# MP-ReID/mp-reid

Hardware: AMD Instinct MI355X
Metric: gallery images/s encode + distmat+rerank ms, 20k×20k; mAP/Rank-1 parity (higher is better)
Workload: dtype f16 pairs hi+lo (3 MFMA products per multiply-add, f32-grade), f32 acc; distmat f32 exact; 1 GPU; Market-1501 configs[1]: do_inference ViT-B/16 3368q+15913g/GPU, no rerank; HBM-resident loader; encoder_batch=508, encoder_precision=split, encoder_streams=2, rerank=False, distance_mode=exact

## Files before the change

mp-reid_amd/csrc/api.cpp:

```cpp
#include "common.h"

#include <cstring>
#include <string>
#include <utility>
#include <vector>

static thread_local char g_err[512] = "";

void mpreid_set_error(const char *fmt, ...) {
    va_list ap;
    va_start(ap, fmt);
    vsnprintf(g_err, sizeof(g_err), fmt, ap);
    va_end(ap);
}

namespace {
struct TuneTable {
    std::vector<std::pair<std::string, int>> kv;
    TuneTable() {
        static const char *known[] = {"gemm_big", "gemm_stagger", "gemm_stagger_all", "jaccard_wave", "jaccard_wave_rows",
                                      "jaccard_table", "csc_atomic", "rerank_overlap", "dist_sym_p2", "dist_sym_p2_naps", "dist_sym_p2_abl", "dist_sym_p2_grid", "dist_sym_p2_strip", "dist_p2_full", "gemm_walk", "gemm_grid", "gemm_ragged", "wide_sort_lds", "wide_jaccard_rows", "verbose"};
        const char *e = getenv("MPREID_TUNE");
        if (!e) return;
        std::string s(e);
        size_t pos = 0;
        while (pos <= s.size()) {
            size_t end = s.find(',', pos);
            if (end == std::string::npos) end = s.size();
            std::string item = s.substr(pos, end - pos);
            pos = end + 1;
            if (item.empty()) continue;
            const size_t eq = item.find('=');
            const std::string key = item.substr(0, eq);
            const int val = eq == std::string::npos ? 1 : atoi(item.c_str() + eq + 1);
            bool ok = false;
            for (const char *k : known) ok = ok || key == k;
            if (!ok) fprintf(stderr, "[mpreid] MPREID_TUNE: unknown key '%s' ignored\n", key.c_str());
            else kv.emplace_back(key, val);
        }
    }
};
}

int mpreid_tune(const char *key, int dflt) {
// ... 41 lines not shown
```

mp-reid_amd/csrc/gemm_f16.hip:

```cpp
#include <algorithm>
#include <cstdlib>
#include <type_traits>

#include "gemm_f16.h"

typedef __attribute__((address_space(3))) void lds_ptr_t;
typedef const __attribute__((address_space(1))) void glb_ptr_t;

__device__ __forceinline__ void dma16(const void *gsrc, unsigned char *lds_dst_wave_base) {
    __builtin_amdgcn_global_load_lds((glb_ptr_t *)gsrc, (lds_ptr_t *)lds_dst_wave_base, 16, 0, 0);
}

__device__ __forceinline__ unsigned lds_addr(const void *p) {
    return (unsigned)(uintptr_t)(const __attribute__((address_space(3))) void *)p;
}
__device__ __forceinline__ void dma16_sv(uint64_t sbase, unsigned voff, unsigned lds_dst) {
    unsigned keep;
    asm volatile("s_mov_b32 %0, m0\n\t"
                 "s_mov_b32 m0, %3\n\t"
                 "s_nop 0\n\t"
                 "global_load_lds_dwordx4 %2, %1 nt\n\t"
                 "s_mov_b32 m0, %0"
                 : "=&s"(keep)
                 : "s"(sbase), "v"(voff), "s"(lds_dst)
// ... 427 lines not shown
                            reinterpret_cast<float *>(g.out)[((int64_t)b * g.L + 1 + p) * g.ldo + n] =
                                a + g.aux[(int64_t)(1 + p) * g.N + n];
                        }
                    } else if (EPI == GE_COSINE) {
                        if (m < g.m_valid && n < g.n_valid) {
                            const float sc = g.rscale ? g.rscale[m] * g.cscale[n] : 1.0f;
                            float c = (a * sc) * __fdiv_rn(1.0f, g.aux[m] * bnv);
                            const float lo = (float)(-1.0 + 0.00001), hi = (float)(1.0 - 0.00001);
                            c = c < lo ? lo : (c > hi ? hi : c);
                            reinterpret_cast<float *>(g.out)[(int64_t)m * g.ldo + n] = acosf(c);
                        }
                    }
                }
        }
    }
}

constexpr int BBM = 256, BBN = 256, BBK = 32, B_NSTAGE = 4;
constexpr int B_PART_BYTES = BBM * BBK * 2;
constexpr int B_STAGE_BYTES = 2 * B_PART_BYTES;
constexpr int B_LDS_BYTES = B_NSTAGE * B_STAGE_BYTES;
constexpr int B_LDS_TOTAL = B_LDS_BYTES + 8 * 4096;

template <int EPI, int DBG = 0, bool SYM = false>
__global__ __launch_bounds__(512) void gemm_f16_big_kernel(GemmArgs g, int tiles_m, int tiles_n) {
    extern __shared__ __attribute__((aligned(16))) unsigned char smem[];
    const int tid = threadIdx.x, lane = tid & 63;
    const int wave = __builtin_amdgcn_readfirstlane(tid >> 6);
    const int wr = wave >> 2, wc = wave & 3;
    const int K = g.K;
    constexpr bool SPLIT = gemm_epi_is_split(EPI);
    constexpr bool SYM_STORE = (EPI == GE_EUCLID) && SYM;
    constexpr bool SYM_EPI = (EPI == GE_CAND) || SYM_STORE;
    const int nseg = SPLIT ? g.kseg / BBK : 0;
    const int nst = SPLIT ? 3 * nseg : K / BBK;
    auto koff_a = [&](int st) -> int {
        if constexpr (!SPLIT) return st * BBK;
        const int r = st / 3, sidx = st - 3 * r;
        return sidx == 0 ? r * BBK : (sidx == 1 ? g.kseg + r * BBK : -1);
    };
    auto koff_b = [&](int st) -> int {
        if constexpr (!SPLIT) return st * BBK;
        const int r = st / 3, sidx = st - 3 * r;
        return sidx == 0 ? r * BBK : (sidx == 2 ? g.kseg + r * BBK : -1);
    };

    const int ntiles = tiles_m * tiles_n;
// ... 179 lines not shown
                const unsigned fl = rw >> 28, row = rw & 0x0fffffffu;
                if (fl & 1u) {
                    const unsigned p = atomicAdd(&g.cnt_lo[row], 1u);
                    if (p < (unsigned)g.cap_lo) g.list_lo[(size_t)row * g.cap_lo + p] = make_uint2(cw, dv);
                }
                if (fl & 2u) {
                    const unsigned p = atomicAdd(&g.cnt_hi[row], 1u);
                    if (p < (unsigned)g.cap_hi) g.list_hi[(size_t)row * g.cap_hi + p] = make_uint2(cw, dv);
                }
                if (fl & 4u) {
                    const unsigned p = atomicAdd(&g.cnt_lo[cw], 1u);
                    if (p < (unsigned)g.cap_lo) g.list_lo[(size_t)cw * g.cap_lo + p] = make_uint2(row, dv);
                }
                if (fl & 8u) {
                    const unsigned p = atomicAdd(&g.cnt_hi[cw], 1u);
                    if (p < (unsigned)g.cap_hi) g.list_hi[(size_t)cw * g.cap_hi + p] = make_uint2(row, dv);
                }
            }
            __builtin_amdgcn_wave_barrier();
            cl_n = 0;
        }
    };

    int tile = tile_at(pos);
    if (tile < 0) return;
    if (g.stagger > 0) {
        const unsigned long long t0 = __builtin_amdgcn_s_memrealtime();
        const unsigned long long wait = g.stagger_mode ? (unsigned long long)g.stagger * ((blockIdx.x >> 3) & 7u) / 8u
                                                       : (unsigned long long)g.stagger * (blockIdx.x & 255u) / 256u;
        while (__builtin_amdgcn_s_memrealtime() - t0 < wait) __builtin_amdgcn_s_sleep(32);
    }
    set_tile(tile);
    dma_prologue();
    [[maybe_unused]] int stamp_tile = 0;
    for (;;) {
    f32x4 acc[8][4];
#pragma unroll
    for (int i = 0; i < 8; ++i)
#pragma unroll
        for (int j = 0; j < 4; ++j) acc[i][j] = f32x4{0.f, 0.f, 0.f, 0.f};

    if constexpr (SPLIT) asm volatile("s_waitcnt vmcnt(4)\n\ts_barrier" ::: "memory");
    else if constexpr (PAIR) {
        if (nst > 2) asm volatile("s_waitcnt vmcnt(8)\n\ts_barrier" ::: "memory");
        else asm volatile("s_waitcnt vmcnt(0)\n\ts_barrier" ::: "memory");
    } else if (nst > 2) asm volatile("s_waitcnt vmcnt(8)\n\ts_barrier" ::: "memory");
    else asm volatile("s_waitcnt vmcnt(4)\n\ts_barrier" ::: "memory");

    auto stamp = [&](int which) {
        if constexpr ((DBG & 32) != 0) {
            if (g.stamps && tid == 0 && stamp_tile < 32)
                g.stamps[((size_t)blockIdx.x * 32 + stamp_tile) * 8 + which] = __builtin_amdgcn_s_memrealtime();
        }
    };
    stamp(0);
    f16x8 fa0[8], fb0[4], fa1[8], fb1[4];
    load_frags(0, fa0, fb0);

    auto mfma32 = [&](f16x8 (&fa)[8], f16x8 (&fb)[4]) {
#pragma unroll
        for (int i = 0; i < 8; ++i)
#pragma unroll
            for (int j = 0; j < 4; ++j)
                acc[i][j] = __builtin_amdgcn_mfma_f32_16x16x32_f16(fa[i], fb[j], acc[i][j], 0, 0, 0);
    };
// ... 55 lines not shown
                else asm volatile("s_waitcnt vmcnt(0)\n\ts_barrier" ::: "memory");
            } else {
                if (t + 2 < nst) asm volatile("s_waitcnt vmcnt(4)\n\ts_barrier" ::: "memory");
                else asm volatile("s_waitcnt vmcnt(0)\n\ts_barrier" ::: "memory");
                if (t + 3 < nst) dma_stage(t + 3);
            }
            load_frags(t + 1, na, nb);
        }
        mfma32(fa, fb);
    };
    if constexpr (SPLIT) {
        auto sstep = [&](auto S_, auto TAIL_, int t) {
            constexpr int S = decltype(S_)::value;
            constexpr bool TAIL = decltype(TAIL_)::value;
            constexpr int s0 = S % 3;
            constexpr bool ldA = s0 != 1, ldB = s0 != 0;
            constexpr bool dmA = s0 != 2, dmB = s0 != 1;
            f16x8 (&fa)[8] = (S & 1) ? fa1 : fa0;
            f16x8 (&fb)[4] = (s0 == 2) ? fb1 : fb0;
            f16x8 (&na)[8] = (S < 3) ? fa1 : fa0;
            f16x8 (&nb)[4] = (s0 == 1) ? fb1 : fb0;
            constexpr bool more1 = !TAIL || S < 5, more3 = !TAIL || S < 3;
            if constexpr (more1) {
                if constexpr (TAIL && S >= 4) asm volatile("s_waitcnt vmcnt(0)\n\ts_barrier" ::: "memory");
                else if constexpr (s0 == 1) asm volatile("s_waitcnt vmcnt(4)\n\ts_barrier" ::: "memory");
                else asm volatile("s_waitcnt vmcnt(2)\n\ts_barrier" ::: "memory");
            }
            unsigned char *dbase = smem + ((t + 3) & (B_NSTAGE - 1)) * B_STAGE_BYTES + wave * 2048;
            const unsigned char *sb = smem + ((t + 1) & (B_NSTAGE - 1)) * B_STAGE_BYTES;
            const int r3 = (t + 3) / 3;
            const int koff = (s0 == 1 ? g.kseg : 0) + r3 * BBK, koffb = (s0 == 2 ? g.kseg : 0) + r3 * BBK;
            auto piece = [&](int q) {
                if (!more3) return;
                if (dmA && q < 2) dma16(a_src + (int64_t)(q * 16) * K + koff, dbase + q * 1024);
                else if (dmB && q - (dmA ? 2 : 0) >= 0 && q - (dmA ? 2 : 0) < 2)
                    dma16(b_src + (int64_t)((q - (dmA ? 2 : 0)) * 16) * K + koffb, dbase + B_PART_BYTES + (q - (dmA ? 2 : 0)) * 1024);
            };
            auto rd_a = [&](int i) { if (more1) na[i] = *reinterpret_cast<const f16x8 *>(sb + a_off + i * 1024); };
            auto rd_b = [&](int j) { if (more1) nb[j] = *reinterpret_cast<const f16x8 *>(sb + b_off + j * 1024); };
#pragma unroll
            for (int gq = 0; gq < 4; ++gq) {
                piece(gq);
                if constexpr (ldA && ldB) {
                    if (gq == 0) { rd_b(0); rd_b(1); rd_b(2); }
                    if (gq == 1) { rd_b(3); rd_a(0); rd_a(1); }
                    if (gq == 2) { rd_a(2); rd_a(3); rd_a(4); }
                    if (gq == 3) { rd_a(5); rd_a(6); rd_a(7); }
// ... 24 lines not shown
        sstep(integral_constant<int, 0>{}, integral_constant<bool, true>{}, t);
        sstep(integral_constant<int, 1>{}, integral_constant<bool, true>{}, t + 1);
        sstep(integral_constant<int, 2>{}, integral_constant<bool, true>{}, t + 2);
        sstep(integral_constant<int, 3>{}, integral_constant<bool, true>{}, t + 3);
        sstep(integral_constant<int, 4>{}, integral_constant<bool, true>{}, t + 4);
        sstep(integral_constant<int, 5>{}, integral_constant<bool, true>{}, t + 5);
    } else {
    int t = 0;
    for (; t + 4 < nst; t += 2) {
        step_steady(std::integral_constant<int, 0>{}, t, fa0, fb0, fa1, fb1);
        step_steady(std::integral_constant<int, 1>{}, t + 1, fa1, fb1, fa0, fb0);
    }
    for (; t < nst; t += 2) {
        step_tail(t, fa0, fb0, fa1, fb1);
        step_tail(t + 1, fa1, fb1, fa0, fb0);
    }
    }

    __syncthreads();
    stamp(1);
    const int cur_m0 = m0, cur_n0 = n0;
    pos += pos_step;
    const int next_tile = tile_at(pos);
    unsigned char *patch = smem + B_LDS_BYTES;
    if constexpr (DBG & 8) {
#pragma unroll
        for (int i = 0; i < 8; ++i)
#pragma unroll
            for (int j = 0; j < 4; ++j) asm volatile("" ::"v"(acc[i][j]));
    } else if constexpr (EPI == GE_CAND) {
        const bool mirror = g.sym != 0 && cur_m0 != cur_n0;
        float *tp = reinterpret_cast<float *>(smem + wave * 16384);
        const int rb = cur_m0 + wr * 128, cb = cur_n0 + wc * 64;
        const float NEG = -__builtin_huge_valf(), POS = __builtin_huge_valf();
        float *rt = tp + 1024;
        float *ct = rt + 384;
        {
            const float a0 = g.aux[rb + lane], a1 = g.aux[rb + 64 + lane];
            const float l0 = g.tlo[rb + lane], l1 = g.tlo[rb + 64 + lane];
            const float h0 = g.thi[rb + lane], h1 = g.thi[rb + 64 + lane];
            const int c = cb + lane;
            const bool cv = c < g.n_valid;
            const float cn = cv ? g.aux2[c] : 0.f;
            const float cl = (mirror && cv) ? g.tlo[c] : NEG, chh = (mirror && cv) ? g.thi[c] : POS;
            rt[lane] = a0; rt[64 + lane] = a1;
            rt[128 + lane] = l0; rt[192 + lane] = l1;
// ... 82 lines not shown
            for (int j = 0; j < 4; ++j)
#pragma unroll
                for (int r = 0; r < 4; ++r) {
                    float v = acc[i][j][r] + bias[j];
                    if (EPI == GE_BIAS_GELU) v = quick_gelu(v);
                    if (EPI == GE_BIAS_RELU) v = v < 0.f ? 0.f : v;
                    wreg[(fq * 4 + r) * 72 + j * 16 + frow] = (_Float16)v;
                }
            __builtin_amdgcn_fence(__ATOMIC_RELEASE, "wavefront");
            __builtin_amdgcn_wave_barrier();
            __builtin_amdgcn_fence(__ATOMIC_ACQUIRE, "wavefront");
#pragma unroll
            for (int it = 0; it < 2; ++it) {
                const int lr = it * 8 + (lane >> 3), ch = lane & 7;
                const uint4 v = *reinterpret_cast<const uint4 *>(wreg + lr * 72 + ch * 8);
                _Float16 *dsth = out + (int64_t)(cur_m0 + wr * 128 + i * 16 + lr) * g.ldo + cur_n0 + wc * 64 + ch * 8;
                if (EPI == GE_BIAS_RELU) *reinterpret_cast<uint4 *>(dsth) = v;
                else store_nt(dsth, v);
            }
            __builtin_amdgcn_wave_barrier();
        }
    } else if constexpr (EPI == GE_S_BIAS_GELU || EPI == GE_S_BIAS_RELU_PAIR) {
        _Float16 *whi = reinterpret_cast<_Float16 *>(patch + wave * 4096);
        _Float16 *wlo = reinterpret_cast<_Float16 *>(smem + wave * 4096);
        _Float16 *out = reinterpret_cast<_Float16 *>(g.out);
        float bias[4];
#pragma unroll
        for (int j = 0; j < 4; ++j) bias[j] = g.bias[cur_n0 + wc * 64 + j * 16 + frow];
#pragma unroll
        for (int i = 0; i < 8; ++i) {
#pragma unroll
            for (int j = 0; j < 4; ++j)
#pragma unroll
                for (int rp = 0; rp < 4; rp += 2) {
                    typedef float f32x2 __attribute__((ext_vector_type(2)));
                    typedef _Float16 f16x2 __attribute__((ext_vector_type(2)));
                    const f32x2 a = {acc[i][j][rp], acc[i][j][rp + 1]};
                    const f32x2 h = __builtin_elementwise_fma(a, f32x2{g.oscale, g.oscale}, f32x2{bias[j], bias[j]});
                    f32x2 v;
                    if constexpr (EPI == GE_S_BIAS_GELU) {
                        const f32x2 t = h * (-1.702f * 1.44269504088896340736f);
                        const f32x2 d = f32x2{__builtin_amdgcn_exp2f(t[0]), __builtin_amdgcn_exp2f(t[1])} + 1.0f;
                        v = h * f32x2{__builtin_amdgcn_rcpf(d[0]), __builtin_amdgcn_rcpf(d[1])};
                    } else {
                        v = f32x2{h[0] < 0.f ? 0.f : h[0], h[1] < 0.f ? 0.f : h[1]};
                    }
                    f16x2 hi, lo;
                    split_pair2(v[0], v[1], hi, lo);
                    whi[(fq * 4 + rp) * 72 + j * 16 + frow] = hi[0];
                    whi[(fq * 4 + rp + 1) * 72 + j * 16 + frow] = hi[1];
                    wlo[(fq * 4 + rp) * 72 + j * 16 + frow] = lo[0];
                    wlo[(fq * 4 + rp + 1) * 72 + j * 16 + frow] = lo[1];
                }
            __builtin_amdgcn_fence(__ATOMIC_RELEASE, "wavefront");
            __builtin_amdgcn_wave_barrier();
            __builtin_amdgcn_fence(__ATOMIC_ACQUIRE, "wavefront");
#pragma unroll
            for (int it = 0; it < 2; ++it) {
                const int lr = it * 8 + (lane >> 3), ch = lane & 7;
                const uint4 vh = *reinterpret_cast<const uint4 *>(whi + lr * 72 + ch * 8);
                const uint4 vl = *reinterpret_cast<const uint4 *>(wlo + lr * 72 + ch * 8);
                _Float16 *dsth = out + (int64_t)(cur_m0 + wr * 128 + i * 16 + lr) * g.ldo + cur_n0 + wc * 64 + ch * 8;
                if constexpr (EPI == GE_S_BIAS_RELU_PAIR) {
                    if (cur_n0 + wc * 64 + ch * 8 < g.pair_c) {
                        *reinterpret_cast<uint4 *>(dsth) = vh;
                        *reinterpret_cast<uint4 *>(dsth + g.pair_c) = vl;
                    }
                } else {
                    store_nt(dsth, vh);
                    store_nt(dsth + g.N, vl);
                }
            }
            __builtin_amdgcn_wave_barrier();
        }
        asm volatile("s_barrier" ::: "memory");
    } else if constexpr (EPI == GE_BIAS_ADD_RELU) {
        _Float16 *wreg = reinterpret_cast<_Float16 *>(patch + wave * 4096);
        _Float16 *pid = reinterpret_cast<_Float16 *>(smem + wave * 4096);
        _Float16 *outh = reinterpret_cast<_Float16 *>(g.out);
        const int nb0 = cur_n0 + wc * 64;
        float bias[4];
#pragma unroll
        for (int j = 0; j < 4; ++j) bias[j] = g.bias[nb0 + j * 16 + frow];
        const int lr0 = lane >> 3, ch = lane & 7;
        auto id_load = [&](int i, int it) -> uint4 {
            return *reinterpret_cast<const uint4 *>(g.identity + (int64_t)(cur_m0 + wr * 128 + i * 16 + it * 8 + lr0) * g.ldo +
                                                    nb0 + ch * 8);
        };
        uint4 idn0 = id_load(0, 0), idn1 = id_load(0, 1);
#pragma unroll
        for (int i = 0; i < 8; ++i) {
            *reinterpret_cast<uint4 *>(pid + lr0 * 72 + ch * 8) = idn0;
            *reinterpret_cast<uint4 *>(pid + (8 + lr0) * 72 + ch * 8) = idn1;
            if (i + 1 < 8) {
                idn0 = id_load(i + 1, 0);
                idn1 = id_load(i + 1, 1);
            }
            __builtin_amdgcn_fence(__ATOMIC_RELEASE, "wavefront");
// ... 91 lines not shown
                store16_sv(x_base(i * 16 + it * 4), x_loff, o);
                if constexpr (EPI == GE_S_BIAS_RES_PAIR) {
                    typedef _Float16 h4p __attribute__((ext_vector_type(4)));
                    h4p hi, lo;
                    {
                        const float y[4] = {o[0] < 0.f ? 0.f : o[0], o[1] < 0.f ? 0.f : o[1], o[2] < 0.f ? 0.f : o[2],
                                            o[3] < 0.f ? 0.f : o[3]};
                        split_pairs<4>(y, hi, lo);
                    }
                    const uint64_t pb = reinterpret_cast<uint64_t>(g.pair_out) +
                                        (uint64_t)(((int64_t)(cur_m0 + wr * 128 + i * 16 + it * 4) * 2 * g.pair_c + nbase) * 2);
                    store8_sv(pb, p_loff, __builtin_bit_cast(u32x2, hi));
                    store8_sv(pb + (uint64_t)g.pair_c * 2u, p_loff, __builtin_bit_cast(u32x2, lo));
                }
            }
            if (i + 4 < 8) x_dma(i + 4);
            __builtin_amdgcn_wave_barrier();
            asm volatile("" ::: "memory");
        }
        asm volatile("s_barrier" ::: "memory");
    } else {
        float *wreg = reinterpret_cast<float *>(patch + wave * 4096);
        float *outp = reinterpret_cast<float *>(g.out);
        const bool vec_ok = (g.ldo % 4 == 0) && ((reinterpret_cast<uintptr_t>(outp) & 15) == 0);
        const int nbase = cur_n0 + wc * 64;
        const int c4 = (lane & 15) * 4;
        float4 bias4 = make_float4(0.f, 0.f, 0.f, 0.f), bn4 = bias4, cs4 = make_float4(1.f, 1.f, 1.f, 1.f);
        float bias1 = 0.f, bnv1 = 0.f, cs1 = 1.f;
        if (EPI == GE_EUCLID && g.rscale) {
            cs4 = *reinterpret_cast<const float4 *>(g.cscale + nbase + c4);
            cs1 = g.cscale[nbase + lane];
        }
        if (vec_ok) {
            if (EPI == GE_BIAS_RES || EPI == GE_S_BIAS_RES || EPI == GE_S_BIAS_RES_PAIR || EPI == GE_S_BIAS_F32)
                bias4 = *reinterpret_cast<const float4 *>(g.bias + nbase + c4);
            if (EPI == GE_EUCLID) {
                bn4.x = (nbase + c4 + 0 < g.n_valid) ? g.aux2[nbase + c4 + 0] : 0.f;
                bn4.y = (nbase + c4 + 1 < g.n_valid) ? g.aux2[nbase + c4 + 1] : 0.f;
                bn4.z = (nbase + c4 + 2 < g.n_valid) ? g.aux2[nbase + c4 + 2] : 0.f;
                bn4.w = (nbase + c4 + 3 < g.n_valid) ? g.aux2[nbase + c4 + 3] : 0.f;
            }
        } else {
            if (EPI == GE_BIAS_RES || EPI == GE_S_BIAS_RES || EPI == GE_S_BIAS_F32) bias1 = g.bias[nbase + lane];
            if (EPI == GE_EUCLID) bnv1 = (nbase + lane < g.n_valid) ? g.aux2[nbase + lane] : 0.f;
        }
        bool fast_path = false;
        if constexpr (EPI == GE_EUCLID || EPI == GE_S_BIAS_F32)
            fast_path = vec_ok && g.ldo < (1 << 24) &&
                        (EPI == GE_S_BIAS_F32 || (cur_m0 + BBM <= g.m_valid && cur_n0 + BBN <= g.n_valid));
        float *rt = fast_path ? reinterpret_cast<float *>(patch + wave * 4096)
                              : reinterpret_cast<float *>(smem + wave * 16384);
        if constexpr (EPI == GE_EUCLID) {
            const int r0 = cur_m0 + wr * 128;
            const float t0 = (r0 + lane < g.m_valid) ? g.aux[r0 + lane] : 0.f;
            const float t1 = (r0 + 64 + lane < g.m_valid) ? g.aux[r0 + 64 + lane] : 0.f;
            float t2 = 1.f, t3 = 1.f;
            if (g.rscale) {
                t2 = g.rscale[r0 + lane];
                t3 = g.rscale[r0 + 64 + lane];
            }
            rt[lane] = t0;
            rt[64 + lane] = t1;
            rt[128 + lane] = t2;
            rt[192 + lane] = t3;
        }
        bool fast_done = false;
        if constexpr (EPI == GE_EUCLID || EPI == GE_S_BIAS_F32) {
            if (fast_path) {
                fast_done = true;
                float *tp4 = reinterpret_cast<float *>(smem + wave * 16384);
                const uint64_t obase = reinterpret_cast<uint64_t>(outp + (int64_t)(cur_m0 + wr * 128) * g.ldo + nbase);
                const unsigned ldo_b = (unsigned)g.ldo * 4u;
                unsigned voff[4];
#pragma unroll
                for (int it = 0; it < 4; ++it) voff[it] = (unsigned)(it * 4 + (lane >> 4)) * ldo_b + (unsigned)c4 * 4u;
                const bool scaled = g.rscale != nullptr;
                #ifndef MPREID_FAST_NBLK
#define MPREID_FAST_NBLK 1
#endif
                constexpr int NBLK = MPREID_FAST_NBLK;
                if constexpr (((DBG >> 7) & 7) == 6) {
#pragma unroll
                    for (int e = 0; e < 32; ++e)
                        store16_nt_sv(obase + (uint64_t)(e >> 2) * 16u * ldo_b, voff[e & 3], acc[e >> 2][e & 3]);
                } else
#pragma unroll
                for (int h = 0; h < 8 / NBLK; ++h) {
#pragma unroll
                    for (int ii = 0; ii < NBLK; ++ii)
#pragma unroll
                        for (int j = 0; j < 4; ++j)
#pragma unroll
                            for (int r = 0; r < 4; ++r)
                                tp4[ii * 1024 + (fq * 4 + r) * 64 + j * 16 + frow] = acc[h * NBLK + ii][j][r];
                    __builtin_amdgcn_fence(__ATOMIC_RELEASE, "wavefront");
                    __builtin_amdgcn_wave_barrier();
                    __builtin_amdgcn_fence(__ATOMIC_ACQUIRE, "wavefront");
                    if (h == 0) stamp(3);
                    float4 av[4 * NBLK];
                    float amv[4 * NBLK], rsv[4 * NBLK];
#pragma unroll
                    for (int e = 0; e < 4 * NBLK; ++e) {
                        const int ii = e >> 2, lr = (e & 3) * 4 + (lane >> 4);
                        av[e] = *reinterpret_cast<const float4 *>(tp4 + ii * 1024 + lr * 64 + c4);
                        if constexpr (EPI == GE_EUCLID) {
                            amv[e] = rt[(h * NBLK + ii) * 16 + lr];
                            rsv[e] = scaled ? rt[128 + (h * NBLK + ii) * 16 + lr] : 1.0f;
                        }
                    }
#pragma unroll
                    for (int e = 0; e < 4 * NBLK; ++e) {
                        const int ii = e >> 2, it = e & 3;
                        const uint64_t pbase = obase + (uint64_t)(h * NBLK + ii) * 16u * ldo_b;
                        const float4 a = av[e];
                        f32x4 o;
                        if constexpr (EPI == GE_S_BIAS_F32) {
                            o[0] = fmaf(a.x, g.oscale, bias4.x);
                            o[1] = fmaf(a.y, g.oscale, bias4.y);
                            o[2] = fmaf(a.z, g.oscale, bias4.z);
                            o[3] = fmaf(a.w, g.oscale, bias4.w);
                        } else if (scaled) {
                            const float rs = rsv[e], am = amv[e];
                            o[0] = fmaf(-2.0f, a.x * (rs * cs4.x), am + bn4.x);
                            o[1] = fmaf(-2.0f, a.y * (rs * cs4.y), am + bn4.y);
                            o[2] = fmaf(-2.0f, a.z * (rs * cs4.z), am + bn4.z);
                            o[3] = fmaf(-2.0f, a.w * (rs * cs4.w), am + bn4.w);
                        } else {
                            const float am = amv[e];
                            o[0] = fmaf(-2.0f, a.x, am + bn4.x);
                            o[1] = fmaf(-2.0f, a.y, am + bn4.y);
                            o[2] = fmaf(-2.0f, a.z, am + bn4.z);
                            o[3] = fmaf(-2.0f, a.w, am + bn4.w);
                        }
                        store16_flav_sv<(DBG >> 7) & 7>(pbase, voff[it], o);
                    }
                    __builtin_amdgcn_wave_barrier();
                    if (h == 0) stamp(6);
                    if (h == 8 / NBLK - 1) stamp(5);
                }
            }
        }
        if (!fast_done) {
#pragma unroll
        for (int i = 0; i < 8; ++i) {
#pragma unroll
            for (int j = 0; j < 4; ++j)
#pragma unroll
                for (int r = 0; r < 4; ++r) wreg[(fq * 4 + r) * 64 + j * 16 + frow] = acc[i][j][r];
            __builtin_amdgcn_fence(__ATOMIC_RELEASE, "wavefront");
            __builtin_amdgcn_wave_barrier();
            __builtin_amdgcn_fence(__ATOMIC_ACQUIRE, "wavefront");
            const int mbase = cur_m0 + wr * 128 + i * 16;
            if (vec_ok) {
#pragma unroll
                for (int it = 0; it < 4; ++it) {
                    const int lr = it * 4 + (lane >> 4);
                    const int m = mbase + lr;
                    const float4 a = *reinterpret_cast<const float4 *>(wreg + lr * 64 + c4);
                    float *dst = outp + (int64_t)m * g.ldo + nbase + c4;
                    if (EPI == GE_F32) {
                        *reinterpret_cast<float4 *>(dst) = a;
                    } else if (EPI == GE_S_BIAS_F32) {
                        store_nt(dst, make_float4(fmaf(a.x, g.oscale, bias4.x), fmaf(a.y, g.oscale, bias4.y),
                                                  fmaf(a.z, g.oscale, bias4.z), fmaf(a.w, g.oscale, bias4.w)));
                    } else if (EPI == GE_S_BIAS_RES) {
// ... 148 lines not shown
                    } else {
#pragma unroll 1
                        for (int e = 0; e < 16; ++e) {
                            const int nl = e * 4 + (lane >> 4);
                            const f32x4 v = *reinterpret_cast<const f32x4 *>(T + nl * 64 + ((l16 ^ (nl & 15)) << 2));
                            const int n = nbase + nl;
                            float *dst = outp + (int64_t)n * g.ldo + mcol;
                            if (n < g.n_valid) {
                                if (vec_ok && mcol + 3 < g.m_valid) {
                                    store_nt(dst, make_float4(v[0], v[1], v[2], v[3]));
                                } else {
                                    if (mcol + 0 < g.m_valid) dst[0] = v[0];
                                    if (mcol + 1 < g.m_valid) dst[1] = v[1];
                                    if (mcol + 2 < g.m_valid) dst[2] = v[2];
                                    if (mcol + 3 < g.m_valid) dst[3] = v[3];
                                }
                            }
                        }
                    }
                    __builtin_amdgcn_wave_barrier();
                }
            }
        }
        if constexpr (EPI == GE_EUCLID || EPI == GE_S_BIAS_F32) asm volatile("s_waitcnt lgkmcnt(0)\n\ts_barrier" ::: "memory");
    }
    stamp(2);
    if constexpr ((DBG & 32) != 0) ++stamp_tile;
    tile = next_tile;
    if (tile < 0) break;
    set_tile(tile);
    dma_prologue();
    }
}

constexpr int PBM = 256, PBN = 128, PBK = 32, P_NSTAGE = 3;
constexpr int P_A_BYTES = PBM * PBK * 2;
constexpr int P_B_BYTES = PBN * PBK * 2;
constexpr int P_STAGE_BYTES = P_A_BYTES + P_B_BYTES;
constexpr int P_RING_BYTES = P_NSTAGE * P_STAGE_BYTES;
constexpr int P_LDS_BYTES = P_RING_BYTES + 4 * 1024;

__device__ __forceinline__ int p2_strip_size(int R, int ncol, int &ramp) {
    ramp = min(ncol, 2 * (R - 1));
    const int p = ramp >> 1;
    return p * (p + 1) + ((ramp & 1) ? (p + 1) : 0) + (ncol - ramp) * R;
}
__device__ __forceinline__ int p2_total_tiles(int tiles_m, int tiles_n, int SH) {
    int T = 0, ramp;
    for (int br = 0; SH * br < tiles_m; ++br) T += p2_strip_size(min(SH, tiles_m - SH * br), tiles_n - 2 * SH * br, ramp);
    return T;
}
__device__ __forceinline__ void p2_tile_at(int k, int tiles_m, int tiles_n, int SH, int &tm, int &tn) {
    int br = 0, R, ramp;
    for (;; ++br) {
// ... 394 lines not shown
                              EPI == GE_EUCLID || EPI == GE_PATCH || EPI == GE_BIAS_RELU || EPI == GE_BIAS_ADD_RELU ||
                              EPI == GE_CAND || gemm_epi_is_split(EPI));
    if constexpr (gemm_epi_is_split(EPI)) {
        if (a.kseg <= 0 || a.kseg % GBK || a.K != 2 * a.kseg) {
            mpreid_set_error("gemm_f16: split epilogue %d needs K == 2 * kseg, kseg a multiple of %d (K=%d kseg=%d)", EPI, GBK,
                             a.K, a.kseg);
            return MPREID_ERR_ARG;
        }
    }
    if constexpr (EPI == GE_CAND) {
        if (a.M % BBM || a.N % BBN) {
            mpreid_set_error("gemm_f16: the candidate epilogue needs M, N multiples of %d", BBM);
            return MPREID_ERR_ARG;
        }
    }
    const int bm = big_mode();
    const bool use_big = HAS_BIG && (EPI == GE_CAND || (bm > 0 && (a.M % BBM == 0) && (a.N % BBN == 0) &&
                                                        (bm >= 2 || (int64_t)(a.M / BBM) * (a.N / BBN) >= 128)));
    if constexpr (HAS_BIG) {
        static PerDeviceOnce big_attr_once;
        const int rc = big_attr_once.run([]() -> int {
            HIP_TRY(hipFuncSetAttribute(reinterpret_cast<const void *>(gemm_f16_big_kernel<EPI>),
                                        hipFuncAttributeMaxDynamicSharedMemorySize, B_LDS_TOTAL));
            return MPREID_OK;
        });
        if (rc) return rc;
    }
    const int tiles_m = use_big ? a.M / BBM : a.M / GBM, tiles_n = use_big ? a.N / BBN : a.N / GBN;
    hipEvent_t e0 = nullptr, e1 = nullptr;
    if (g_prof_on) {
        HIP_TRY(hipEventCreate(&e0));
        HIP_TRY(hipEventCreate(&e1));
        HIP_TRY(hipEventRecord(e0, stream));
    }
    bool use_p2 = false, p2_full = false;
    if constexpr (EPI == GE_EUCLID) {
        static const int p2_mode = mpreid_tune("dist_sym_p2", 1);
        use_p2 = a.sym && p2_mode > 0 && a.M == a.N && (a.A == a.W || p2_mode >= 3) && (a.M % PBM == 0) && (a.K % PBK == 0) &&
                 (p2_mode >= 2 || a.M / PBM >= 16);
        static const int full_mode = mpreid_tune("dist_p2_full", 0);
        if (!use_p2 && !a.sym && full_mode > 0 && a.out && (a.M % PBM == 0) && (a.N % PBN == 0) && (a.K % PBK == 0) &&
            (full_mode >= 2 || (a.M / PBM >= 16 && a.N / PBN >= 32)))
            use_p2 = p2_full = true;
    }
    if (use_p2) {
        if constexpr (EPI == GE_EUCLID) {
// ... 53 lines not shown
        if constexpr (HAS_BIG) {
            static const int dbg = mpreid_ablation_env("MPREID_GEMM_DBG");
            int big_cus = 0;
            if (const int rcc = current_device_cus(&big_cus)) return rcc;
            static const int stag_all = mpreid_tune("gemm_stagger_all", 0);
            static const int walk_tune = mpreid_tune("gemm_walk", -1);
            GemmArgs a = a_in;
            if (stag_all > 0) {
                a.stagger = stag_all;
                a.stagger_mode = 1;
            }
            a.walk = walk_tune >= 3 ? walk_tune
                   : (walk_tune == 2 || (walk_tune == 1 && tiles_n <= 4) || (walk_tune < 0 && tiles_n <= 4 && (int64_t)a.K * 2 >= 8192)) ? 1 : 0;
            if (walk_tune < 3 && tiles_m % 64 != 0 && tiles_m % 32 == 0) a.walk |= 8;
            static const int ragged_tune = mpreid_tune("gemm_ragged", 1);
            if (!ragged_tune) a.walk |= 16;
            const unsigned total_tiles = (unsigned)tiles_m * (unsigned)tiles_n;
#ifdef MPREID_ABLATION
            if (const char *gg = getenv("MPREID_GEMM_GRID")) big_cus = atoi(gg);
#endif
            static const int grid_tune = mpreid_tune("gemm_grid", 0);
            if (grid_tune > 0 && grid_tune < big_cus) big_cus = grid_tune;
            const dim3 grid(total_tiles < (unsigned)big_cus ? total_tiles : (unsigned)big_cus);
#ifdef MPREID_ABLATION
            if (dbg == 64 && gemm_epi_is_split(EPI)) {
                HIP_TRY(hipFuncSetAttribute(reinterpret_cast<const void *>(gemm_f16_big_kernel<EPI, 64>),
                                            hipFuncAttributeMaxDynamicSharedMemorySize, B_LDS_TOTAL));
                hipLaunchKernelGGL((gemm_f16_big_kernel<EPI, 64>), grid, dim3(512), B_LDS_TOTAL, stream, a, tiles_m, tiles_n);
            } else if (dbg == 32 && EPI != GE_EUCLID && EPI != GE_BIAS_GELU) {
                GemmArgs as = a;
                const char *sp = getenv("MPREID_GEMM_STAMPS");
                as.stamps = sp ? reinterpret_cast<unsigned long long *>(strtoull(sp, nullptr, 16)) : nullptr;
                HIP_TRY(hipFuncSetAttribute(reinterpret_cast<const void *>(gemm_f16_big_kernel<EPI, 32>),
                                            hipFuncAttributeMaxDynamicSharedMemorySize, B_LDS_TOTAL));
                hipLaunchKernelGGL((gemm_f16_big_kernel<EPI, 32>), grid, dim3(512), B_LDS_TOTAL, stream, as, tiles_m, tiles_n);
            } else
#endif
            if constexpr (EPI == GE_BIAS_F16) {
#define MPREID_DBG_CASE(D)                                                                                  \
    case D: {                                                                                               \
        HIP_TRY(hipFuncSetAttribute(reinterpret_cast<const void *>(gemm_f16_big_kernel<EPI, D>),            \
                                    hipFuncAttributeMaxDynamicSharedMemorySize, B_LDS_TOTAL));              \
        hipLaunchKernelGGL((gemm_f16_big_kernel<EPI, D>), grid, dim3(512), B_LDS_TOTAL, stream, a, tiles_m, tiles_n); \
        break;                                                                                              \
    }
                switch (dbg) {
                    MPREID_DBG_CASE(1) MPREID_DBG_CASE(2) MPREID_DBG_CASE(3) MPREID_DBG_CASE(4) MPREID_DBG_CASE(5)
                    MPREID_DBG_CASE(7) MPREID_DBG_CASE(8) MPREID_DBG_CASE(9) MPREID_DBG_CASE(15) MPREID_DBG_CASE(16)
                    MPREID_DBG_CASE(24)
                default:
                    hipLaunchKernelGGL(gemm_f16_big_kernel<EPI>, grid, dim3(512), B_LDS_TOTAL, stream, a, tiles_m, tiles_n);
                }
#undef MPREID_DBG_CASE
            } else if constexpr (EPI == GE_EUCLID || EPI == GE_BIAS_GELU) {
                if (dbg == 800) {
                    GemmArgs as = a;
                    const char *sp = getenv("MPREID_GEMM_STAMPS");
                    as.stamps = sp ? reinterpret_cast<unsigned long long *>(strtoull(sp, nullptr, 16)) : nullptr;
                    HIP_TRY(hipFuncSetAttribute(reinterpret_cast<const void *>(gemm_f16_big_kernel<EPI, 800>),
                                                hipFuncAttributeMaxDynamicSharedMemorySize, B_LDS_TOTAL));
                    hipLaunchKernelGGL((gemm_f16_big_kernel<EPI, 800>), grid, dim3(512), B_LDS_TOTAL, stream, as, tiles_m, tiles_n);
// ... 309 lines not shown
```

Before: 16950 images/s.

## Prefetch next tile's first K-stages during split-GEMM epilogue

Adds an EARLY variant of the persistent big GEMM kernel for the split-precision bias and bias-GELU epilogues. It issues the next tile's first three DMA stages before the epilogue stores, overlapping global loads with the epilogue. It pads the vmcnt counter with dummy bias loads so the waitcnt counts stay uniform, and reworks the epilogue LDS staging to fit above the ring. This aims to hide the per-tile pipeline refill bubble, at the cost of intricate hand-counted waitcnt logic and reduced LDS slack.

Result: no change. 17040 images/s (median of 4 runs) (+0.5%).

```diff
diff --git a/mp-reid_amd/csrc/api.cpp b/mp-reid_amd/csrc/api.cpp
--- a/mp-reid_amd/csrc/api.cpp
+++ b/mp-reid_amd/csrc/api.cpp
@@ -19,7 +19,7 @@
     std::vector<std::pair<std::string, int>> kv;
     TuneTable() {
         static const char *known[] = {"gemm_big", "gemm_stagger", "gemm_stagger_all", "jaccard_wave", "jaccard_wave_rows",
-                                      "jaccard_table", "csc_atomic", "rerank_overlap", "dist_sym_p2", "dist_sym_p2_naps", "dist_sym_p2_abl", "dist_sym_p2_grid", "dist_sym_p2_strip", "dist_p2_full", "gemm_walk", "gemm_grid", "gemm_ragged", "wide_sort_lds", "wide_jaccard_rows", "verbose"};
+                                      "jaccard_table", "csc_atomic", "rerank_overlap", "dist_sym_p2", "dist_sym_p2_naps", "dist_sym_p2_abl", "dist_sym_p2_grid", "dist_sym_p2_strip", "dist_p2_full", "gemm_walk", "gemm_grid", "gemm_ragged", "gemm_early", "wide_sort_lds", "wide_jaccard_rows", "verbose"};
         const char *e = getenv("MPREID_TUNE");
         if (!e) return;
         std::string s(e);
diff --git a/mp-reid_amd/csrc/gemm_f16.hip b/mp-reid_amd/csrc/gemm_f16.hip
--- a/mp-reid_amd/csrc/gemm_f16.hip
+++ b/mp-reid_amd/csrc/gemm_f16.hip
@@ -473,7 +473,7 @@
 constexpr int B_LDS_BYTES = B_NSTAGE * B_STAGE_BYTES;
 constexpr int B_LDS_TOTAL = B_LDS_BYTES + 8 * 4096;
 
-template <int EPI, int DBG = 0, bool SYM = false>
+template <int EPI, int DBG = 0, bool SYM = false, bool EARLY = false>
 __global__ __launch_bounds__(512) void gemm_f16_big_kernel(GemmArgs g, int tiles_m, int tiles_n) {
     extern __shared__ __attribute__((aligned(16))) unsigned char smem[];
     const int tid = threadIdx.x, lane = tid & 63;
@@ -699,6 +699,21 @@
         }
     };
 
+    constexpr bool EARLY_EPI = EARLY && (EPI == GE_S_BIAS_F32 || EPI == GE_S_BIAS_GELU);
+    constexpr int E_NPRE = 3;
+    constexpr int E_STORES = 32;
+    [[maybe_unused]] int next_tile_e = -1;
+    auto early_prefetch = [&]() {
+        if constexpr (EARLY_EPI) {
+            if (next_tile_e >= 0) {
+                set_tile(next_tile_e);
+                asm volatile("" : "+v"(a_src), "+v"(b_src)::"memory");
+#pragma unroll
+                for (int st = 0; st < E_NPRE; ++st) dma_stage(st);
+            }
+        }
+    };
+
     int tile = tile_at(pos);
     if (tile < 0) return;
     if (g.stagger > 0) {
@@ -708,7 +723,15 @@
         while (__builtin_amdgcn_s_memrealtime() - t0 < wait) __builtin_amdgcn_s_sleep(32);
     }
     set_tile(tile);
-    dma_prologue();
+    if constexpr (EARLY_EPI) {
+#pragma unroll
+        for (int st = 0; st < E_NPRE; ++st) dma_stage(st);
+#pragma unroll
+        for (int e = 0; e < E_STORES; ++e)
+            __builtin_amdgcn_global_load_lds((glb_ptr_t *)(g.bias + lane), (lds_ptr_t *)(smem + B_LDS_BYTES + wave * 4096), 4, 0, 0);
+    } else {
+        dma_prologue();
+    }
     [[maybe_unused]] int stamp_tile = 0;
     for (;;) {
     f32x4 acc[8][4];
@@ -717,7 +740,12 @@
 #pragma unroll
         for (int j = 0; j < 4; ++j) acc[i][j] = f32x4{0.f, 0.f, 0.f, 0.f};
 
-    if constexpr (SPLIT) asm volatile("s_waitcnt vmcnt(4)\n\ts_barrier" ::: "memory");
+    if constexpr (EARLY_EPI) {
+        static_assert(E_NPRE == 3, "the counts below are written for the early stages 0-2");
+        constexpr int TOPW = 2 + 2 + E_STORES;
+        static_assert(TOPW <= 63, "vmcnt is a 6-bit counter");
+        asm volatile("s_waitcnt vmcnt(%0)\n\ts_barrier" ::"n"(TOPW) : "memory");
+    } else if constexpr (SPLIT) asm volatile("s_waitcnt vmcnt(4)\n\ts_barrier" ::: "memory");
     else if constexpr (PAIR) {
         if (nst > 2) asm volatile("s_waitcnt vmcnt(8)\n\ts_barrier" ::: "memory");
         else asm volatile("s_waitcnt vmcnt(0)\n\ts_barrier" ::: "memory");
@@ -819,7 +847,19 @@
             f16x8 (&nb)[4] = (s0 == 1) ? fb1 : fb0;
             constexpr bool more1 = !TAIL || S < 5, more3 = !TAIL || S < 3;
             if constexpr (more1) {
-                if constexpr (TAIL && S >= 4) asm volatile("s_waitcnt vmcnt(0)\n\ts_barrier" ::: "memory");
+                if constexpr (EARLY_EPI && S + 1 < E_NPRE) {
+                    constexpr int NW = (s0 == 1) ? 4 : 2;
+                    constexpr int FW = NW + E_STORES;
+                    static_assert(FW <= 63, "vmcnt is a 6-bit counter");
+                    asm volatile("s_cmp_eq_u32 %0, %1\n\t"
+                                 "s_cbranch_scc1 1f\n\t"
+                                 "s_waitcnt vmcnt(%2)\n\t"
+                                 "s_branch 2f\n"
+                                 "1:\n\t"
+                                 "s_waitcnt vmcnt(%3)\n"
+                                 "2:\n\t"
+                                 "s_barrier" ::"s"(t), "n"(S), "n"(NW), "n"(FW) : "memory", "scc");
+                } else if constexpr (TAIL && S >= 4) asm volatile("s_waitcnt vmcnt(0)\n\ts_barrier" ::: "memory");
                 else if constexpr (s0 == 1) asm volatile("s_waitcnt vmcnt(4)\n\ts_barrier" ::: "memory");
                 else asm volatile("s_waitcnt vmcnt(2)\n\ts_barrier" ::: "memory");
             }
@@ -890,6 +930,7 @@
     const int cur_m0 = m0, cur_n0 = n0;
     pos += pos_step;
     const int next_tile = tile_at(pos);
+    if constexpr (EARLY_EPI) next_tile_e = next_tile;
     unsigned char *patch = smem + B_LDS_BYTES;
     if constexpr (DBG & 8) {
 #pragma unroll
@@ -1018,11 +1059,23 @@
         }
     } else if constexpr (EPI == GE_S_BIAS_GELU || EPI == GE_S_BIAS_RELU_PAIR) {
         _Float16 *whi = reinterpret_cast<_Float16 *>(patch + wave * 4096);
-        _Float16 *wlo = reinterpret_cast<_Float16 *>(smem + wave * 4096);
+        _Float16 *wlo = reinterpret_cast<_Float16 *>(smem + (EARLY_EPI ? 3 * B_STAGE_BYTES : 0) + wave * 4096);
         _Float16 *out = reinterpret_cast<_Float16 *>(g.out);
+        int el = lane;
+        if constexpr (EARLY_EPI) asm volatile("" : "+v"(el));
+        const int efrow = el & 15, efq = el >> 4;
         float bias[4];
 #pragma unroll
-        for (int j = 0; j < 4; ++j) bias[j] = g.bias[cur_n0 + wc * 64 + j * 16 + frow];
+        for (int j = 0; j < 4; ++j) bias[j] = g.bias[cur_n0 + wc * 64 + j * 16 + efrow];
+        [[maybe_unused]] unsigned hi_addr = 0, lo_addr = 0, st_voff = 0;
+        if constexpr (EARLY_EPI) {
+            asm volatile("" : "+v"(bias[0]), "+v"(bias[1]), "+v"(bias[2]), "+v"(bias[3])::"memory");
+            early_prefetch();
+            const unsigned poff = (unsigned)((el >> 3) * 72 + (el & 7) * 8) * 2u;
+            hi_addr = lds_addr(whi) + poff;
+            lo_addr = lds_addr(wlo) + poff;
+            st_voff = ((unsigned)(el >> 3) * (unsigned)g.ldo + (unsigned)(el & 7) * 8u) * 2u;
+        }
 #pragma unroll
         for (int i = 0; i < 8; ++i) {
 #pragma unroll
@@ -1043,11 +1096,33 @@
                     }
                     f16x2 hi, lo;
                     split_pair2(v[0], v[1], hi, lo);
-                    whi[(fq * 4 + rp) * 72 + j * 16 + frow] = hi[0];
-                    whi[(fq * 4 + rp + 1) * 72 + j * 16 + frow] = hi[1];
-                    wlo[(fq * 4 + rp) * 72 + j * 16 + frow] = lo[0];
-                    wlo[(fq * 4 + rp + 1) * 72 + j * 16 + frow] = lo[1];
-                }
+                    whi[(efq * 4 + rp) * 72 + j * 16 + efrow] = hi[0];
+                    whi[(efq * 4 + rp + 1) * 72 + j * 16 + efrow] = hi[1];
+                    wlo[(efq * 4 + rp) * 72 + j * 16 + efrow] = lo[0];
+                    wlo[(efq * 4 + rp + 1) * 72 + j * 16 + efrow] = lo[1];
+                }
+            if constexpr (EARLY_EPI) {
+                asm volatile("" ::: "memory");
+                __builtin_amdgcn_wave_barrier();
+                f32x4 vh0, vh1, vl0, vl1;
+                asm volatile("ds_read_b128 %0, %4\n\t"
+                             "ds_read_b128 %1, %4 offset:1152\n\t"
+                             "ds_read_b128 %2, %5\n\t"
+                             "ds_read_b128 %3, %5 offset:1152\n\t"
+                             "s_waitcnt lgkmcnt(0)"
+                             : "=&v"(vh0), "=&v"(vh1), "=&v"(vl0), "=&v"(vl1)
+                             : "v"(hi_addr), "v"(lo_addr)
+                             : "memory");
+                const uint64_t sb0 = reinterpret_cast<uint64_t>(out + (int64_t)(cur_m0 + wr * 128 + i * 16) * g.ldo + cur_n0 + wc * 64);
+                const uint64_t sb1 = sb0 + (uint64_t)g.ldo * 16u;
+                store16_nt_sv(sb0, st_voff, vh0);
+                store16_nt_sv(sb0 + (uint64_t)g.N * 2u, st_voff, vl0);
+                store16_nt_sv(sb1, st_voff, vh1);
+                store16_nt_sv(sb1 + (uint64_t)g.N * 2u, st_voff, vl1);
+                __builtin_amdgcn_wave_barrier();
+                asm volatile("" ::: "memory");
+                continue;
+            }
             __builtin_amdgcn_fence(__ATOMIC_RELEASE, "wavefront");
             __builtin_amdgcn_wave_barrier();
             __builtin_amdgcn_fence(__ATOMIC_ACQUIRE, "wavefront");
@@ -1069,7 +1144,7 @@
             }
             __builtin_amdgcn_wave_barrier();
         }
-        asm volatile("s_barrier" ::: "memory");
+        if constexpr (!EARLY_EPI) asm volatile("s_barrier" ::: "memory");
     } else if constexpr (EPI == GE_BIAS_ADD_RELU) {
         _Float16 *wreg = reinterpret_cast<_Float16 *>(patch + wave * 4096);
         _Float16 *pid = reinterpret_cast<_Float16 *>(smem + wave * 4096);
@@ -1207,9 +1282,12 @@
     } else {
         float *wreg = reinterpret_cast<float *>(patch + wave * 4096);
         float *outp = reinterpret_cast<float *>(g.out);
-        const bool vec_ok = (g.ldo % 4 == 0) && ((reinterpret_cast<uintptr_t>(outp) & 15) == 0);
+        const bool vec_ok = EARLY_EPI || ((g.ldo % 4 == 0) && ((reinterpret_cast<uintptr_t>(outp) & 15) == 0));
         const int nbase = cur_n0 + wc * 64;
-        const int c4 = (lane & 15) * 4;
+        int el = lane;
+        if constexpr (EARLY_EPI) asm volatile("" : "+v"(el));
+        const int efrow = el & 15, efq = el >> 4;
+        const int c4 = (el & 15) * 4;
         float4 bias4 = make_float4(0.f, 0.f, 0.f, 0.f), bn4 = bias4, cs4 = make_float4(1.f, 1.f, 1.f, 1.f);
         float bias1 = 0.f, bnv1 = 0.f, cs1 = 1.f;
         if (EPI == GE_EUCLID && g.rscale) {
@@ -1229,8 +1307,8 @@
             if (EPI == GE_BIAS_RES || EPI == GE_S_BIAS_RES || EPI == GE_S_BIAS_F32) bias1 = g.bias[nbase + lane];
             if (EPI == GE_EUCLID) bnv1 = (nbase + lane < g.n_valid) ? g.aux2[nbase + lane] : 0.f;
         }
-        bool fast_path = false;
-        if constexpr (EPI == GE_EUCLID || EPI == GE_S_BIAS_F32)
+        bool fast_path = EARLY_EPI;
+        if constexpr (!EARLY_EPI && (EPI == GE_EUCLID || EPI == GE_S_BIAS_F32))
             fast_path = vec_ok && g.ldo < (1 << 24) &&
                         (EPI == GE_S_BIAS_F32 || (cur_m0 + BBM <= g.m_valid && cur_n0 + BBN <= g.n_valid));
         float *rt = fast_path ? reinterpret_cast<float *>(patch + wave * 4096)
@@ -1253,12 +1331,21 @@
         if constexpr (EPI == GE_EUCLID || EPI == GE_S_BIAS_F32) {
             if (fast_path) {
                 fast_done = true;
-                float *tp4 = reinterpret_cast<float *>(smem + wave * 16384);
+                if constexpr (EARLY_EPI) {
+                    asm volatile("" : "+v"(bias4.x), "+v"(bias4.y), "+v"(bias4.z), "+v"(bias4.w)::"memory");
+                    early_prefetch();
+                }
+                float *tp4 = EARLY_EPI ? reinterpret_cast<float *>(patch + wave * 4096)
+                                       : reinterpret_cast<float *>(smem + wave * 16384);
+                [[maybe_unused]] unsigned tp_addr = 0;
+                if constexpr (EARLY_EPI) {
+                    tp_addr = lds_addr(tp4) + (unsigned)el * 16u;
+                }
                 const uint64_t obase = reinterpret_cast<uint64_t>(outp + (int64_t)(cur_m0 + wr * 128) * g.ldo + nbase);
                 const unsigned ldo_b = (unsigned)g.ldo * 4u;
                 unsigned voff[4];
 #pragma unroll
-                for (int it = 0; it < 4; ++it) voff[it] = (unsigned)(it * 4 + (lane >> 4)) * ldo_b + (unsigned)c4 * 4u;
+                for (int it = 0; it < 4; ++it) voff[it] = (unsigned)(it * 4 + (el >> 4)) * ldo_b + (unsigned)c4 * 4u;
                 const bool scaled = g.rscale != nullptr;
                 #ifndef MPREID_FAST_NBLK
 #define MPREID_FAST_NBLK 1
@@ -1277,16 +1364,37 @@
                         for (int j = 0; j < 4; ++j)
 #pragma unroll
                             for (int r = 0; r < 4; ++r)
-                                tp4[ii * 1024 + (fq * 4 + r) * 64 + j * 16 + frow] = acc[h * NBLK + ii][j][r];
-                    __builtin_amdgcn_fence(__ATOMIC_RELEASE, "wavefront");
-                    __builtin_amdgcn_wave_barrier();
-                    __builtin_amdgcn_fence(__ATOMIC_ACQUIRE, "wavefront");
+                                tp4[ii * 1024 + (efq * 4 + r) * 64 + j * 16 + efrow] = acc[h * NBLK + ii][j][r];
+                    if constexpr (EARLY_EPI) {
+                        asm volatile("" ::: "memory");
+                        __builtin_amdgcn_wave_barrier();
+                    } else {
+                        __builtin_amdgcn_fence(__ATOMIC_RELEASE, "wavefront");
+                        __builtin_amdgcn_wave_barrier();
+                        __builtin_amdgcn_fence(__ATOMIC_ACQUIRE, "wavefront");
+                    }
                     if (h == 0) stamp(3);
                     float4 av[4 * NBLK];
                     float amv[4 * NBLK], rsv[4 * NBLK];
+                    if constexpr (EARLY_EPI) {
+                        static_assert(!EARLY_EPI || NBLK == 1, "the early prologue has room for one patch above the ring");
+                        f32x4 r0, r1, r2, r3;
+                        asm volatile("ds_read_b128 %0, %4\n\t"
+                                     "ds_read_b128 %1, %4 offset:1024\n\t"
+                                     "ds_read_b128 %2, %4 offset:2048\n\t"
+                                     "ds_read_b128 %3, %4 offset:3072\n\t"
+                                     "s_waitcnt lgkmcnt(0)"
+                                     : "=&v"(r0), "=&v"(r1), "=&v"(r2), "=&v"(r3)
+                                     : "v"(tp_addr)
+                                     : "memory");
+                        av[0] = make_float4(r0[0], r0[1], r0[2], r0[3]);
+                        av[1] = make_float4(r1[0], r1[1], r1[2], r1[3]);
+                        av[2] = make_float4(r2[0], r2[1], r2[2], r2[3]);
+                        av[3] = make_float4(r3[0], r3[1], r3[2], r3[3]);
+                    } else
 #pragma unroll
                     for (int e = 0; e < 4 * NBLK; ++e) {
-                        const int ii = e >> 2, lr = (e & 3) * 4 + (lane >> 4);
+                        const int ii = e >> 2, lr = (e & 3) * 4 + (el >> 4);
                         av[e] = *reinterpret_cast<const float4 *>(tp4 + ii * 1024 + lr * 64 + c4);
                         if constexpr (EPI == GE_EUCLID) {
                             amv[e] = rt[(h * NBLK + ii) * 16 + lr];
@@ -1325,7 +1433,7 @@
                 }
             }
         }
-        if (!fast_done) {
+        if (!EARLY_EPI && !fast_done) {
 #pragma unroll
         for (int i = 0; i < 8; ++i) {
 #pragma unroll
@@ -1520,14 +1628,18 @@
                 }
             }
         }
-        if constexpr (EPI == GE_EUCLID || EPI == GE_S_BIAS_F32) asm volatile("s_waitcnt lgkmcnt(0)\n\ts_barrier" ::: "memory");
+        if constexpr (EARLY_EPI) {
+            if (!fast_path) asm volatile("s_waitcnt lgkmcnt(0)\n\ts_barrier" ::: "memory");
+        } else if constexpr (EPI == GE_EUCLID || EPI == GE_S_BIAS_F32) asm volatile("s_waitcnt lgkmcnt(0)\n\ts_barrier" ::: "memory");
     }
     stamp(2);
     if constexpr ((DBG & 32) != 0) ++stamp_tile;
     tile = next_tile;
     if (tile < 0) break;
-    set_tile(tile);
-    dma_prologue();
+    if constexpr (!EARLY_EPI) {
+        set_tile(tile);
+        dma_prologue();
+    }
     }
 }
 
@@ -1968,6 +2080,9 @@
         const int rc = big_attr_once.run([]() -> int {
             HIP_TRY(hipFuncSetAttribute(reinterpret_cast<const void *>(gemm_f16_big_kernel<EPI>),
                                         hipFuncAttributeMaxDynamicSharedMemorySize, B_LDS_TOTAL));
+            if constexpr (EPI == GE_S_BIAS_F32 || EPI == GE_S_BIAS_GELU)
+                HIP_TRY(hipFuncSetAttribute(reinterpret_cast<const void *>(gemm_f16_big_kernel<EPI, 0, false, true>),
+                                            hipFuncAttributeMaxDynamicSharedMemorySize, B_LDS_TOTAL));
             return MPREID_OK;
         });
         if (rc) return rc;
@@ -2067,6 +2182,9 @@
             static const int grid_tune = mpreid_tune("gemm_grid", 0);
             if (grid_tune > 0 && grid_tune < big_cus) big_cus = grid_tune;
             const dim3 grid(total_tiles < (unsigned)big_cus ? total_tiles : (unsigned)big_cus);
+            static const int early_tune = mpreid_tune("gemm_early", 1);
+            [[maybe_unused]] const bool early_ok = early_tune != 0 &&
+                (EPI != GE_S_BIAS_F32 || (a.ldo % 4 == 0 && (reinterpret_cast<uintptr_t>(a.out) & 15) == 0 && a.ldo < (1 << 24)));
 #ifdef MPREID_ABLATION
             if (dbg == 64 && gemm_epi_is_split(EPI)) {
                 HIP_TRY(hipFuncSetAttribute(reinterpret_cast<const void *>(gemm_f16_big_kernel<EPI, 64>),
@@ -2078,10 +2196,22 @@
                 as.stamps = sp ? reinterpret_cast<unsigned long long *>(strtoull(sp, nullptr, 16)) : nullptr;
                 HIP_TRY(hipFuncSetAttribute(reinterpret_cast<const void *>(gemm_f16_big_kernel<EPI, 32>),
                                             hipFuncAttributeMaxDynamicSharedMemorySize, B_LDS_TOTAL));
+                if constexpr (EPI == GE_S_BIAS_F32 || EPI == GE_S_BIAS_GELU) {
+                    if (early_ok) {
+                        HIP_TRY(hipFuncSetAttribute(reinterpret_cast<const void *>(gemm_f16_big_kernel<EPI, 32, false, true>),
+                                                    hipFuncAttributeMaxDynamicSharedMemorySize, B_LDS_TOTAL));
+                        hipLaunchKernelGGL((gemm_f16_big_kernel<EPI, 32, false, true>), grid, dim3(512), B_LDS_TOTAL, stream, as, tiles_m, tiles_n);
+                    } else {
+                        hipLaunchKernelGGL((gemm_f16_big_kernel<EPI, 32>), grid, dim3(512), B_LDS_TOTAL, stream, as, tiles_m, tiles_n);
+                    }
+                } else
                 hipLaunchKernelGGL((gemm_f16_big_kernel<EPI, 32>), grid, dim3(512), B_LDS_TOTAL, stream, as, tiles_m, tiles_n);
             } else
 #endif
-            if constexpr (EPI == GE_BIAS_F16) {
+            if constexpr (EPI == GE_S_BIAS_F32 || EPI == GE_S_BIAS_GELU) {
+                if (early_ok) hipLaunchKernelGGL((gemm_f16_big_kernel<EPI, 0, false, true>), grid, dim3(512), B_LDS_TOTAL, stream, a, tiles_m, tiles_n);
+                else hipLaunchKernelGGL(gemm_f16_big_kernel<EPI>, grid, dim3(512), B_LDS_TOTAL, stream, a, tiles_m, tiles_n);
+            } else if constexpr (EPI == GE_BIAS_F16) {
 #define MPREID_DBG_CASE(D)                                                                                  \
     case D: {                                                                                               \
         HIP_TRY(hipFuncSetAttribute(reinterpret_cast<const void *>(gemm_f16_big_kernel<EPI, D>),            \
```
